# nordmtr/quantpy

Hardware: AMD Instinct MI355X
Metric: state reconstructions/sec (3-qubit MLE) (higher is better)
Workload: dtype f64

## Files before the change

quantpy_amd/csrc/qt_small.h:

```cpp
#pragma once
#include <hip/hip_runtime.h>
#include <stdint.h>

#include <type_traits>

#include "qt_linesearch.h"

namespace qt {

#ifdef QT_PHASE_TIMING
__device__ long long* g_qt_prof = nullptr;
#define QT_STAMP(slot)                                                                                   \
  do {                                                                                                   \
    if (g_qt_prof && (threadIdx.x & 63) == 0)                                                            \
      g_qt_prof[((size_t)blockIdx.x * (blockDim.x >> 6) + (threadIdx.x >> 6)) * 32 + (slot)] =           \
          (long long)__builtin_readcyclecounter();                                                       \
  } while (0)
#define QT_STAMP_VAL(slot, val)                                                                          \
  do {                                                                                                   \
    if (g_qt_prof && (threadIdx.x & 63) == 0)                                                            \
      g_qt_prof[((size_t)blockIdx.x * (blockDim.x >> 6) + (threadIdx.x >> 6)) * 32 + (slot)] = (val);    \
  } while (0)
#else
#define QT_STAMP(slot) do {} while (0)
#define QT_STAMP_VAL(slot, val) do {} while (0)
#endif

struct alignas(16) cd {
  double re, im;
};
__device__ __forceinline__ cd cmul(cd a, cd b) { return {a.re * b.re - a.im * b.im, a.re * b.im + a.im * b.re}; }
__device__ __forceinline__ cd cmulc(cd a, cd b) {
  return {a.re * b.re + a.im * b.im, a.im * b.re - a.re * b.im};
}
__device__ __forceinline__ cd cadd(cd a, cd b) { return {a.re + b.re, a.im + b.im}; }
__device__ __forceinline__ cd hs_term(cd a, cd b) {
  return {__builtin_fma(a.re, b.re, -(a.im * b.im)), __builtin_fma(a.re, b.im, a.im * b.re)};
}
__device__ __forceinline__ cd cscale(cd a, double s) { return {a.re * s, a.im * s}; }

__device__ __forceinline__ void wave_sync() {
  __builtin_amdgcn_wave_barrier();
  asm volatile("" ::: "memory");
}

template <int CTRL, int ROW_MASK = 0xf>
__device__ __forceinline__ double dpp_f64(double v) {
  const long long b = __builtin_bit_cast(long long, v);
  const int lo = __builtin_amdgcn_update_dpp(0, (int)(b & 0xffffffffLL), CTRL, ROW_MASK, 0xf, ROW_MASK == 0xf);
  const int hi = __builtin_amdgcn_update_dpp(0, (int)(b >> 32), CTRL, ROW_MASK, 0xf, ROW_MASK == 0xf);
  return __builtin_bit_cast(double, ((long long)hi << 32) | (unsigned int)lo);
}
__device__ __forceinline__ double readlane_f64(double v, int lane) {
  const long long b = __builtin_bit_cast(long long, v);
  const int lo = __builtin_amdgcn_readlane((int)(b & 0xffffffffLL), lane);
  const int hi = __builtin_amdgcn_readlane((int)(b >> 32), lane);
  return __builtin_bit_cast(double, ((long long)hi << 32) | (unsigned int)lo);
}
__device__ __forceinline__ double nanmax(double a, double b) { return (b > a || b != b) ? b : a; }

template <int G>
__device__ __forceinline__ double gsum(double v) {
  v += dpp_f64<0xB1>(v);
  v += dpp_f64<0x4E>(v);
  if (G >= 8) v += dpp_f64<0x141>(v);
  if (G >= 16) v += dpp_f64<0x140>(v);
  if (G == 64) {
    v += dpp_f64<0x142, 0xA>(v);
    v += dpp_f64<0x143, 0xC>(v);
    v = readlane_f64(v, 63);
  }
  return v;
}
template <int G>
__device__ __forceinline__ bool group_any(bool pred) {
  const unsigned long long votes = __builtin_amdgcn_ballot_w64(pred);
  if (G == 64) return votes != 0ull;
  const int lane = threadIdx.x & 63;
  return (votes & (((1ull << (G & 63)) - 1ull) << (lane / G * G))) != 0ull;
}
__device__ __forceinline__ double max_f64(double a, double b) {
  double r;
  asm("v_max_f64 %0, %1, %2" : "=v"(r) : "v"(a), "v"(b));
  return r;
}
template <int G>
__device__ __forceinline__ double gmax(double v) {
  const bool nan = group_any<G>(v != v);
  v = max_f64(v, dpp_f64<0xB1>(v));
  v = max_f64(v, dpp_f64<0x4E>(v));
  if (G >= 8) v = max_f64(v, dpp_f64<0x141>(v));
  if (G >= 16) v = max_f64(v, dpp_f64<0x140>(v));
  if (G == 64) {
    v = max_f64(v, dpp_f64<0x142, 0xA>(v));
    v = max_f64(v, dpp_f64<0x143, 0xC>(v));
    v = readlane_f64(v, 63);
  }
  return nan ? __builtin_nan("") : v;
}

__device__ __forceinline__ double recip_nr(double x) {
  double r = __builtin_amdgcn_rcp(x);
  r = fma(r, fma(-x, r, 1.0), r);
  return fma(r, fma(-x, r, 1.0), r);
}
__device__ __forceinline__ bool log_is_regular(double x) { return x > 0.0 && x < 1.7e308; }
__device__ __forceinline__ double fast_log(double x) {
  if (!(x > 0.0) || !(x < 1.7e308)) return x == 0.0 ? -__builtin_huge_val() : (x > 0.0 ? x : __builtin_nan(""));
  double m = __builtin_amdgcn_frexp_mant(x);
  int e = __builtin_amdgcn_frexp_exp(x);
  const bool low = m < 0.70710678118654752440;
  m = low ? m + m : m;
  e = low ? e - 1 : e;
  const double num = m - 1.0, den = m + 1.0;
  const double r = recip_nr(den);
  double sq = num * r;
  sq = fma(r, fma(-sq, den, num), sq);
  const double z = sq * sq;
  const double z2 = z * z, z4 = z2 * z2, z8 = z4 * z4;
  const double q0 = fma(z, 1.0 / 5.0, 1.0 / 3.0), q1 = fma(z, 1.0 / 9.0, 1.0 / 7.0);
  const double q2 = fma(z, 1.0 / 13.0, 1.0 / 11.0), q3 = fma(z, 1.0 / 17.0, 1.0 / 15.0);
  const double q4 = fma(z, 1.0 / 21.0, 1.0 / 19.0);
  const double r0 = fma(z2, q1, q0), r1 = fma(z2, q3, q2);
  const double pl = fma(z8, q4, fma(z4, r1, r0));
  const double lm = fma(sq + sq, pl * z, sq + sq);
  const double ed = (double)e;
  return fma(ed, 6.93147180369123816490e-01, fma(ed, 1.90821492927058770002e-10, lm));
}

constexpr bool kLiftSingleNegative = true;

__device__ __forceinline__ double fast_rsqrt(double x) {
  double y = __builtin_amdgcn_rsq(x);
  double e = fma(-x * y, y, 1.0);
  y = fma(y * e, fma(e, 0.375, 0.5), y);
  e = fma(-x * y, y, 1.0);
  return fma(y * e, 0.5, y);
}

template <int UNR>
__device__ __forceinline__ void dot_block(const double* __restrict__ base, size_t stride, unsigned lane_off,
                                          const double* lds_vec, int m, double (&acc)[4]) {
  double av[UNR];
#pragma unroll
  for (int u = 0; u < UNR; ++u) av[u] = base[(size_t)(m + u) * stride + lane_off];
#pragma unroll
  for (int u = 0; u < UNR; ++u) acc[u & 3] = fma(av[u], lds_vec[m + u], acc[u & 3]);
  __builtin_amdgcn_sched_group_barrier(0x020, UNR, 0);
#pragma unroll
  for (int u = 0; u < UNR; u += 4) {
    __builtin_amdgcn_sched_group_barrier(0x100, 2, 0);
    __builtin_amdgcn_sched_group_barrier(0x002, 4, 0);
  }
}
template <int UNR>
__device__ __forceinline__ double dot_global(const double* __restrict__ base, size_t stride, unsigned lane_off,
                                             const double* lds_vec, int n) {
  double acc[4] = {0.0, 0.0, 0.0, 0.0};
  int m = 0;
  for (; m + UNR <= n; m += UNR) dot_block<UNR>(base, stride, lane_off, lds_vec, m, acc);
  if (UNR > 8 && m + 8 <= n) {
    dot_block<8>(base, stride, lane_off, lds_vec, m, acc);
    m += 8;
  }
  if (UNR > 4 && m + 4 <= n) {
    dot_block<4>(base, stride, lane_off, lds_vec, m, acc);
    m += 4;
  }
  for (; m < n; ++m) acc[0] = fma(base[(size_t)m * stride + lane_off], lds_vec[m], acc[0]);
  return (acc[0] + acc[1]) + (acc[2] + acc[3]);
}

__device__ __forceinline__ void rotation(double app, double aqq, cd apq, double& cs, cd& w) {
  const double ab2 = apq.re * apq.re + apq.im * apq.im;
  cs = 1.0;
  w = cd{0.0, 0.0};
  if (ab2 > 1e-300) {
    const double dl = 0.5 * (aqq - app);
    const double x = fma(dl, dl, ab2);
    double y = __builtin_amdgcn_rsq(x);
    y = fma(y * fma(-x * y, y, 1.0), 0.5, y);
    const double den = fabs(dl) + x * y;
    double z = __builtin_amdgcn_rcp(den);
    z = fma(z, fma(-den, z, 1.0), z);
    const double u = copysign(z, dl);
    cs = fast_rsqrt(fma(u * u, ab2, 1.0));
    const double cu = cs * u;
    w = cd{cu * apq.re, cu * apq.im};
  }
}


struct ProductView {
  const double* T;
  const double* P1T;
  const double* wrowR;
  const int* rmap;
  const int* rinv;
  const int* fwd;
  const int* bwd;
  int R1;
  int uniform;
  double wuni;
  int enabled;
  int pairedT, pairedP;
  double cT[12], cP[12];
  const int* last;
};

struct PovmView {
  const double* Aw;
  const double* AwT;
  const double* PinvT;
  int M;
  ProductView pr;
  double jtol2 = 1e-28;
  const double* Ns = nullptr;
  int S = 0, K = 0;
  double ns_tot = 0.0;
  int extra = 0;
};

struct SpecArgs {
  const void* image;
  const double* Ns;
  double ns_tot, wuni, jtol2;
  int M, extra;
  double cT[12], cP[12];
};
template <bool GENERIC>
struct MleArgs {
  using type = PovmView;
};
template <>
struct MleArgs<false> {
  using type = SpecArgs;
};

__device__ __forceinline__ bool shots_match(double t_s, double total, double n_s, double ns_tot) {
  const double a = t_s * ns_tot, b = n_s * total;
  return fabs(a - b) <= 2e-15 * fabs(b);
}

struct EstOut {
  double* rho;
  const double* centre;
  double* dist;
};

template <int NQ>
struct Small {
  static constexpr int d = 1 << NQ;
  static constexpr int D = d * d;
  static constexpr int G = D;
  static constexpr int TPW = 64 / G;
  static constexpr int WPB = 4;
  static constexpr int NT = 64 * WPB;
  static constexpr int TPB = TPW * WPB;
  static constexpr int T = d * (d - 1) / 2;
  static constexpr int LD = d == 8 ? 9 : d;
  static constexpr int MAT = 2 * LD * d;
  static constexpr int oA = 0;
  static constexpr int oB = oA + MAT;
  static constexpr int oVec = oB + MAT;
  static constexpr int oLam = oVec + D + 2;
  static constexpr int oM = oLam + 2 * ((d + 1) / 2);
  __host__ __device__ static bool v_on_rbuf(int M) { return ((M + 1) & ~1) >= MAT; }
  __host__ __device__ static int v_offset(int M, int R1) {
    const int Mp = (M + 1) & ~1;
    return v_on_rbuf(M) ? oM : oM + (R1 > 0 ? 3 : 2) * Mp;
  }
  __host__ __device__ static int trial_doubles(int M, int R1 = 0) {
    const int Mp = (M + 1) & ~1;
    return oM + (R1 > 0 ? 3 : 2) * Mp + (v_on_rbuf(M) ? 0 : MAT);
  }
  __host__ __device__ static int ipow_h(int b, int e) {
    int r = 1;
    for (int t = 0; t < e; ++t) r *= b;
    return r;
  }
  __host__ __device__ static int fwd_ints(int R1) {
    int t = 0;
    for (int q = 1; q <= NQ; ++q) t += ipow_h(R1, q) << (2 * (NQ - q));
    return t;
  }
  __host__ __device__ static int bwd_ints(int R1) {
    int t = 0;
    for (int q = 1; q <= NQ; ++q) t += ipow_h(R1, q - 1) << (2 * (NQ - q + 1));
    return t;
  }
  __host__ __device__ static int table_ints(int M, int R1) { return (fwd_ints(R1) + bwd_ints(R1) + M + 1) & ~1; }
  __host__ __device__ static int table_doubles(int M, int R1) {
    return R1 > 0 ? (table_ints(M, R1) / 2 + ((M + 1) & ~1) + 8 * R1) : 0;
  }
  __host__ __device__ static size_t lds_bytes(int M, int R1 = 0, int extra = 0) {
    return ((size_t)table_doubles(M, R1) + (size_t)TPB * (trial_doubles(M, R1) + extra)) * sizeof(double);
  }

  struct Ctx {
    int l, i, j, e;
    double* sm;
    const int *tfwd, *tbwd, *trmap;
    const double* twrow;
    const double *ttab, *ptab;
    int M, Mp;
    PovmView pv;
    int xm, zm, ny;
    int pi, pj, pkind;
    int src_re, src_im;
    __device__ __forceinline__ cd* A() const { return reinterpret_cast<cd*>(sm + oA); }
    __device__ __forceinline__ cd* Bm() const { return reinterpret_cast<cd*>(sm + oB); }
    __device__ __forceinline__ cd* V() const { return reinterpret_cast<cd*>(sm + v_offset(M, pv.pr.enabled ? pv.pr.R1 : 0)); }
    __device__ __forceinline__ double* vec() const { return sm + oVec; }
    __device__ __forceinline__ double* lam() const { return sm + oLam; }
    __device__ __forceinline__ double* rbuf() const { return sm + oM; }
    __device__ __forceinline__ double* freq() const { return sm + oM + Mp; }
    __device__ __forceinline__ double* bufB() const { return sm + oM + 2 * Mp; }
    __device__ __forceinline__ const double* tabT() const { return ttab; }
    __device__ __forceinline__ const double* tabP() const { return ptab; }
    __device__ __forceinline__ bool prod() const { return pv.pr.enabled != 0; }
    __device__ __forceinline__ double* extra() const { return sm + trial_doubles(M, pv.pr.enabled ? pv.pr.R1 : 0); }
    static constexpr bool kGeneric = true;
    static constexpr bool kHelper = false;
    __device__ __forceinline__ int R1() const { return pv.pr.R1; }
    __device__ __forceinline__ bool uniform() const { return pv.pr.uniform != 0; }
    __device__ __forceinline__ bool pairedT() const { return pv.pr.pairedT != 0; }
    __device__ __forceinline__ bool pairedP() const { return pv.pr.pairedP != 0; }
    __device__ __forceinline__ double wuni() const { return pv.pr.wuni; }
    __device__ __forceinline__ double jtol2() const { return pv.jtol2; }
    __device__ __forceinline__ double cT(int k) const { return pv.pr.cT[k]; }
    __device__ __forceinline__ double cP(int k) const { return pv.pr.cP[k]; }
  };
  struct CtxS {
    int l, i, j, e;
    double* sm;
    const int* tfwd;
    const double *ttab, *ptab;
    int M, Mp;
    SpecArgs a;
    int xm, zm, ny;
    int pi, pj, pkind;
    int src_re, src_im;
    int bslot;
    double kT[12], kP[12];
    __device__ __forceinline__ cd* A() const { return reinterpret_cast<cd*>(sm + oA); }
    __device__ __forceinline__ cd* Bm() const { return reinterpret_cast<cd*>(sm + oB); }
    __device__ __forceinline__ cd* V() const { return reinterpret_cast<cd*>(sm + v_offset(M, 6)); }
    __device__ __forceinline__ double* vec() const { return sm + oVec; }
    __device__ __forceinline__ double* lam() const { return sm + oLam; }
    __device__ __forceinline__ double* rbuf() const { return sm + oM; }
    __device__ __forceinline__ double* freq() const { return sm + oM + Mp; }
    __device__ __forceinline__ double* bufB() const { return sm + oM + 2 * Mp; }
    __device__ __forceinline__ const double* tabT() const { return ttab; }
    __device__ __forceinline__ const double* tabP() const { return ptab; }
    __device__ __forceinline__ double* extra() const { return sm + trial_doubles(M, 6); }
    static constexpr bool kGeneric = false;
    static constexpr bool kHelper = false;
    __device__ __forceinline__ static constexpr bool prod() { return true; }
    __device__ __forceinline__ static constexpr int R1() { return 6; }
    __device__ __forceinline__ static constexpr bool uniform() { return true; }
    __device__ __forceinline__ static constexpr bool pairedT() { return true; }
    __device__ __forceinline__ static constexpr bool pairedP() { return true; }
    __device__ __forceinline__ double wuni() const { return a.wuni; }
    __device__ __forceinline__ double jtol2() const { return a.jtol2; }
    __device__ __forceinline__ double cT(int k) const { return kT[k]; }
    __device__ __forceinline__ double cP(int k) const { return kP[k]; }
  };
  __device__ __forceinline__ static double pin_vgpr(double x) {
    asm volatile("" : "+v"(x));
    return x;
  }
  template <bool GENERIC, class = void>
  struct CtxOf {
    using type = Ctx;
  };
  template <class X>
  struct CtxOf<false, X> {
    using type = CtxS;
  };
  __host__ __device__ static int image_last_ints(int M) { return (M + 3) & ~3; }
  __host__ __device__ static int image_chunks(int M) { return image_last_ints(M) / 4 + 2 * 24 / 2; }

  __device__ __forceinline__ static int trial_index(int B, bool* live) {
    const int wave = threadIdx.x >> 6, tib = (threadIdx.x & 63) / G;
    const int b = (blockIdx.x * WPB + wave) * TPW + tib;
    *live = b < B;
    return b;
  }

  __device__ static void make_ctx(Ctx& c, double* smem_block, const PovmView& pv) {
    const int lane = threadIdx.x & 63, wave = threadIdx.x >> 6;
    c.l = lane % G;
    const int slot = wave * TPW + lane / G;
    c.i = c.l / d;
    c.j = c.l % d;
    c.e = c.i * LD + c.j;
    c.M = pv.M;
    c.Mp = (pv.M + 1) & ~1;
    c.pv = pv;
    const int r1 = pv.pr.enabled ? pv.pr.R1 : 0;
    int* tabs = reinterpret_cast<int*>(smem_block);
    c.tfwd = tabs;
    c.tbwd = tabs + fwd_ints(r1);
    c.trmap = c.tbwd + bwd_ints(r1);
    double* wrow = smem_block + table_ints(pv.M, r1) / 2;
    double* t1 = wrow + ((pv.M + 1) & ~1);
    c.twrow = wrow;
    c.ttab = t1;
    c.ptab = t1 + 4 * r1;
    if (r1 > 0) {
      const int nf = fwd_ints(r1), nb = bwd_ints(r1);
      for (int e = threadIdx.x; e < 4 * r1; e += NT) {
        t1[e] = pv.pr.T[e];
        t1[4 * r1 + e] = pv.pr.P1T[e];
      }
      if (pv.pr.pairedT) {
        for (int e = threadIdx.x; e < pv.M; e += NT) tabs[e] = pv.pr.last[e];
      } else {
        for (int e = threadIdx.x; e < nf; e += NT) tabs[e] = pv.pr.fwd[e];
      }
      if (!(pv.pr.pairedT && pv.pr.pairedP))
        for (int e = threadIdx.x; e < nb; e += NT) tabs[nf + e] = pv.pr.bwd[e];
      for (int e = threadIdx.x; e < pv.M; e += NT) {
        tabs[nf + nb + e] = pv.pr.rmap[e];
        wrow[e] = pv.pr.wrowR[e];
      }
      __syncthreads();
    }
    c.sm = smem_block + table_doubles(pv.M, r1) + slot * (trial_doubles(pv.M, r1) + pv.extra);
    int xm = 0, zm = 0, ny = 0;
#pragma unroll
    for (int b = 0; b < NQ; ++b) {
      const int dig = (c.l >> (2 * b)) & 3;
      if (dig == 1 || dig == 2) xm |= 1 << b;
      if (dig == 2 || dig == 3) zm |= 1 << b;
      if (dig == 2) ++ny;
    }
    c.xm = xm;
    c.zm = zm;
    c.ny = ny & 3;
    if (c.l < d) {
      c.pi = c.pj = c.l;
      c.pkind = 0;
    } else {
      int t = c.l - d;
      c.pkind = 1;
      if (t >= T) {
        t -= T;
        c.pkind = 2;
      }
      int ii = 1;
      while ((ii * (ii + 1)) / 2 <= t) ++ii;
      c.pi = ii;
      c.pj = t - (ii * (ii - 1)) / 2;
    }
    c.src_re = c.src_im = D;
    if (c.i == c.j) c.src_re = c.i;
    else if (c.i > c.j) {
      const int tt = (c.i * (c.i - 1)) / 2 + c.j;
      c.src_re = d + tt;
      c.src_im = d + T + tt;
    }
    if (c.l == 0) c.sm[oVec + D] = 0.0;
  }

  __device__ __forceinline__ static int pauli_index(int x, int z) {
    int k = 0;
#pragma unroll
    for (int b = 0; b < NQ; ++b) {
      const int xb = (x >> b) & 1, zb = (z >> b) & 1;
      const int dig = xb ? (zb ? 2 : 1) : (zb ? 3 : 0);
      k |= dig << (2 * b);
    }
    return k;
  }
  __device__ __forceinline__ static double re_phase(int ny, cd s) {
    return ny == 0 ? s.re : ny == 1 ? s.im : ny == 2 ? -s.re : -s.im;
  }
  __device__ __forceinline__ static cd phase_times(int ny, double v) {
    return ny == 0 ? cd{v, 0.0} : ny == 1 ? cd{0.0, -v} : ny == 2 ? cd{-v, 0.0} : cd{0.0, v};
  }

  __device__ __forceinline__ static cd wht_step(cd s, cd p, bool upper) {
    return upper ? cd{p.re - s.re, p.im - s.im} : cd{s.re + p.re, s.im + p.im};
  }
  template <class C>
  __device__ static double bloch_of(const C& c, const cd* m) {
    if constexpr (NQ == 3) {
      const int x = c.i, r = c.j, lane = threadIdx.x & 63;
      const cd e = m[r * LD + (r ^ x)];
      cd s{e.re, -e.im};
      s = wht_step(s, cd{dpp_f64<0xB1>(s.re), dpp_f64<0xB1>(s.im)}, lane & 1);
      s = wht_step(s, cd{dpp_f64<0x4E>(s.re), dpp_f64<0x4E>(s.im)}, lane & 2);
      s = wht_step(s, cd{__shfl_xor(s.re, 4), __shfl_xor(s.im, 4)}, lane & 4);
      const int z = r;
      const double v = re_phase(__popc(x & z) & 3, s) / d;
      const int sx = (x & 1) | ((x & 2) << 1) | ((x & 4) << 2), sz = (z & 1) | ((z & 2) << 1) | ((z & 4) << 2);
      double* vec = c.vec();
      if constexpr (C::kGeneric) vec[sx ^ (3 * sz)] = v;
      else vec[c.bslot] = v;
      wave_sync();
      const double mine = vec[c.l];
      wave_sync();
      return mine;
    }
    cd s{0.0, 0.0};
#pragma unroll
    for (int r = 0; r < d; ++r) {
      const cd e = m[r * LD + (r ^ c.xm)];
      const double sg = (__popc(r & c.zm) & 1) ? -1.0 : 1.0;
// ... 464 lines not shown
    return dot_global<(D < 16 ? D : 16)>(g_transposed, (size_t)c.M, (unsigned)row, vec, D);
  }

  template <class C>
  __device__ static cd lin_invert(const C& c, double& bloch_l) {
    if constexpr (!C::kGeneric) {
      bloch_l = prod_backward<true>(c, c.freq()) / (c.wuni() * d);
    } else if (c.prod()) {
      if (c.uniform()) {
        bloch_l = prod_backward<true>(c, c.freq()) / (c.wuni() * d);
      } else {
        double acc = 0.0;
        for (int m = 0; m < c.M; ++m) acc = fma(c.pv.PinvT[(size_t)c.trmap[m] * D + c.l], c.freq()[m], acc);
        bloch_l = acc / d;
      }
    } else {
      bloch_l = col_dot(c, c.pv.PinvT, c.freq()) / d;
    }
    c.vec()[c.l] = bloch_l;
    wave_sync();
    cd r = matrix_of(c, c.vec());
    wave_sync();
    return r;
  }

  template <class C>
  __device__ static cd psd_project(const C& c, cd a, double eps) {
    const int i = c.i, j = c.j;
    cd* Ai = c.A();
    cd* Vi = c.V();
    cd v{i == j ? 1.0 : 0.0, 0.0};
    if (i == j) a.im = 0.0;
    const double nrm = gsum<G>(a.re * a.re + a.im * a.im);
    for (int sweep = 0; sweep < 20; ++sweep) {
      const double off = gsum<G>(i != j ? a.re * a.re + a.im * a.im : 0.0);
      if (__all(!(off > c.jtol2() * nrm))) break;
#pragma unroll 1
      for (int r = 1; r < d; ++r) {
        Ai[c.e] = a;
        Vi[c.e] = v;
        wave_sync();
        const int pj = j ^ r, pi = i ^ r;
        const int cp = j < pj ? j : pj, cq = j < pj ? pj : j;
        const int rp = i < pi ? i : pi, rq = i < pi ? pi : i;
        const double c_pp = Ai[cp * LD + cp].re, c_qq = Ai[cq * LD + cq].re;
        const cd c_pq = Ai[cp * LD + cq];
        const double r_pp = Ai[rp * LD + rp].re, r_qq = Ai[rq * LD + rq].re;
        const cd r_pq = Ai[rp * LD + rq];
        const cd a_c = Ai[i * LD + pj], a_r = Ai[pi * LD + j], a_x = Ai[pi * LD + pj];
        const cd v_c = Vi[i * LD + pj];
        wave_sync();
        double cj, ci;
        cd wj, wi;
        rotation(c_pp, c_qq, c_pq, cj, wj);
        rotation(r_pp, r_qq, r_pq, ci, wi);
        if (j < pj) wj = cd{-wj.re, wj.im};
        if (i < pi) wi = cd{-wi.re, wi.im};
        const cd t0 = cadd(cscale(a, cj), cmul(a_c, wj));
        const cd t1 = cadd(cscale(a_r, cj), cmul(a_x, wj));
        a = cadd(cscale(t0, ci), cmulc(t1, wi));
        v = cadd(cscale(v, cj), cmul(v_c, wj));
        if (i == j) a.im = 0.0;
      }
    }
    double* lam = c.lam();
    Vi[c.e] = v;
    if (i == j) lam[i] = a.re;
    wave_sync();
    cd rr{0.0, 0.0};
#pragma unroll
    for (int k = 0; k < d; ++k) {
      const double lc = lam[k] > eps ? lam[k] : eps;
      const cd p = cmulc(Vi[i * LD + k], Vi[j * LD + k]);
      rr.re += lc * p.re;
      rr.im += lc * p.im;
    }
    const double tr = gsum<G>(i == j ? rr.re : 0.0);
    wave_sync();
    return cd{rr.re / tr, rr.im / tr};
  }

  template <bool SPEC = false, class C>
  __device__ static double cholesky_param(const C& c, cd a, int& ok, int* neg_out = nullptr, int* kneg_out = nullptr,
                                          cd* spec_inv = nullptr) {
    cd* A = c.A();
    cd* L = c.Bm();
    cd* Vs = c.V();
    const int i = c.i, j = c.j;
    A[c.e] = a;
    int neg = 0, kneg = d - 1;
    cd lmine{0.0, 0.0};
    cd b = a;
    if (SPEC && i == j) b.im = 0.0;
    if (SPEC) Vs[c.e] = b;
    wave_sync();
#pragma unroll
    for (int k = 0; k < d; ++k) {
      const double akk = (G == 64) ? readlane_f64(a.re, k * d + k) : A[k * LD + k].re;
      const cd aik = A[i * LD + k], ajk = A[j * LD + k];
      if constexpr (SPEC) {
        const double piv = readlane_f64(b.re, k * d + k);
        const cd bip = Vs[i * LD + k], bpj = Vs[k * LD + j];
        double inv = __builtin_amdgcn_rcp(piv);
        inv = fma(inv, fma(-piv, inv, 1.0), inv);
        inv = fma(inv, fma(-piv, inv, 1.0), inv);
        const cd t{bpj.re * inv, bpj.im * inv};
        const cd e = cmul(bip, t);
        cd nb{b.re - e.re, b.im - e.im};
        if (j == k) nb = cd{-bip.re * inv, -bip.im * inv};
        if (i == k) nb = (j == k) ? cd{inv, 0.0} : t;
        b = nb;
        if (k + 1 < d) Vs[c.e] = b;
      }
      const double mag = fabs(akk);
      const bool pos = akk > 0.0;
      if (!pos) {
        if (neg == 0) kneg = k;
        ++neg;
      }
      if (!(mag > 1e-13)) neg = neg > 0 ? 99 : neg;
      const double safe = mag > 1e-300 ? mag : 1e-300;
      if (k + 1 < d) {
        const double inv = recip_nr(safe);
        const double sinv = pos ? -inv : inv;
        const cd ajs{ajk.re * sinv, ajk.im * sinv};
        const bool upd = i > k && j > k;
        const double nre = fma(aik.re, ajs.re, fma(aik.im, ajs.im, a.re));
        const double nim = fma(aik.im, ajs.re, fma(-aik.re, ajs.im, a.im));
        a.re = upd ? nre : a.re;
        a.im = upd ? nim : a.im;
        A[c.e] = a;
        wave_sync();
      }
    }
    {
      const double dj = A[j * LD + j].re;
      const double mj = fabs(dj);
      const double rs = fast_rsqrt(mj > 1e-300 ? mj : 1e-300);
      if (i >= j) lmine = (i == j) ? cd{dj * rs, 0.0} : cd{a.re * rs, a.im * rs};
    }
    ok = neg == 0;
    if (neg_out) *neg_out = neg;
    if (kneg_out) *kneg_out = kneg;
    if (SPEC && spec_inv) *spec_inv = b;
    L[c.e] = lmine;
    wave_sync();
    const cd e = L[c.pi * LD + c.pj];
    const double x = c.pkind == 2 ? e.im : e.re;
    wave_sync();
    return x;
  }

  struct HelperLink {
    enum : int { kNone = 0, kSweep = 1, kUnset = 2, kClaimed = 3, kRevoked = 4 };
    static constexpr int kHelperPolls = 1 << 15, kWaitPolls = 1 << 12, kClaimedPolls = 1 << 16;
    double* base;
    int pending;
    __device__ __forceinline__ static constexpr int doubles() { return MAT + D + 2; }
    __device__ __forceinline__ cd* image() const { return reinterpret_cast<cd*>(base); }
    __device__ __forceinline__ double* x() const { return base + MAT; }
    __device__ __forceinline__ int* task() const { return reinterpret_cast<int*>(base + MAT + D); }
    __device__ __forceinline__ int* done() const { return task() + 1; }
    __device__ __forceinline__ int* ok() const { return task() + 2; }
    __device__ __forceinline__ static void publish(int* w, int v) {
      wave_sync();
      if ((threadIdx.x & 63) == 0) __hip_atomic_store(w, v, __ATOMIC_RELEASE, __HIP_MEMORY_SCOPE_WORKGROUP);
    }
    __device__ __forceinline__ static int peek(const int* w) {
      return __builtin_amdgcn_readfirstlane(__hip_atomic_load(w, __ATOMIC_RELAXED, __HIP_MEMORY_SCOPE_WORKGROUP));
    }
    __device__ __forceinline__ static bool claim(int* w, int to) {
      int won = 0;
      if ((threadIdx.x & 63) == 0) {
        int expect = kSweep;
        won = __hip_atomic_compare_exchange_strong(w, &expect, to, __ATOMIC_ACQ_REL, __ATOMIC_RELAXED,
                                                   __HIP_MEMORY_SCOPE_WORKGROUP);
      }
      return __builtin_amdgcn_readfirstlane(won) != 0;
    }
    template <int SLEEP>
    __device__ __forceinline__ static int poll(const int* w, int idle, int polls) {
      int v = idle;
#pragma unroll 1
      for (int n = 0; n < polls; ++n) {
        v = peek(w);
        if (v != idle) break;
        __builtin_amdgcn_s_sleep(SLEEP);
      }
      return v;
    }
    __device__ __forceinline__ void reset() {
      pending = 0;
      if ((threadIdx.x & 63) == 0) {
        *task() = kUnset;
        *done() = 0;
      }
    }
    __device__ __forceinline__ void none() const { publish(task(), kNone); }
    __device__ __forceinline__ void give(int e, cd proj) {
      image()[e] = proj;
      publish(task(), kSweep);
      pending = 1;
    }
    __device__ __forceinline__ bool collect(int l, double& xl, int& okl) const {
      if (poll<1>(done(), 0, kWaitPolls) == 0) {
        if (claim(task(), kRevoked)) return false;
        if (poll<1>(done(), 0, kClaimedPolls) == 0) return false;
      }
      __builtin_amdgcn_fence(__ATOMIC_ACQUIRE, "workgroup");
      xl = x()[l];
      okl = *ok();
      return true;
    }
  };
  struct CtxH {
    int l, i, j, e, pi, pj, pkind;
    cd *image, *factor;
    __device__ __forceinline__ cd* A() const { return image; }
    __device__ __forceinline__ cd* Bm() const { return factor; }
    __device__ __forceinline__ cd* V() const { return nullptr; }
  };
  struct LateX {
    bool got;
    double x;
    int ok;
  };
  template <class Base>
  struct WithHelper : Base {
    HelperLink* link;
    LateX* late;
    static constexpr bool kHelper = true;
  };
  __device__ __forceinline__ static void param_owner(int l, int& pi, int& pj, int& pkind) {
    const bool diag = l < d, imag = l >= d + T;
    const int t = l - d - (imag ? T : 0);
    int ii = 1;
#pragma unroll
    for (int k = 2; k < d; ++k) ii += t >= (k * (k - 1)) / 2;
    pkind = diag ? 0 : imag ? 2 : 1;
    pi = diag ? l : ii;
    pj = diag ? l : t - (ii * (ii - 1)) / 2;
  }
  __device__ static void helper_wave(const HelperLink& k, cd* L) {
    static_assert(G == 64, "one trial per wavefront");
    if (HelperLink::template poll<2>(k.task(), HelperLink::kUnset, HelperLink::kHelperPolls) != HelperLink::kSweep) return;
    if (!HelperLink::claim(k.task(), HelperLink::kClaimed)) return;
    __builtin_amdgcn_fence(__ATOMIC_ACQUIRE, "workgroup");
    CtxH c;
    c.l = threadIdx.x & 63;
    c.i = c.l / d;
    c.j = c.l % d;
    c.e = c.i * LD + c.j;
    param_owner(c.l, c.pi, c.pj, c.pkind);
    c.image = k.image();
    c.factor = L;
    int ok2;
    const double x2 = cholesky_param(c, c.image[c.e], ok2);
    k.x()[c.l] = x2;
    if (c.l == 0) *k.ok() = ok2;
    HelperLink::publish(k.done(), 1);
  }

  template <class C>
  __device__ static bool lift_single_negative(const C& c, cd r, int kneg, double eps, cd& out,
                                              const cd* inverse = nullptr) {
    static_assert(G == 64, "one trial per wavefront: the flags below are wave-uniform");
    cd* Ai = c.A();
    cd* Vi = c.V();
    const int i = c.i, j = c.j;
    if (i == j) r.im = 0.0;
    cd b = r;
    if (inverse) b = *inverse;
#pragma unroll 1
    for (int s = inverse ? d : 0; s < d; ++s) {
      const int p = s < kneg ? s : (s < d - 1 ? s + 1 : kneg);
      Ai[c.e] = b;
      const double piv = readlane_f64(b.re, p * d + p);
      wave_sync();
      const cd bip = Ai[i * LD + p], bpj = Ai[p * LD + j];
      wave_sync();
      double inv = __builtin_amdgcn_rcp(piv);
      inv = fma(inv, fma(-piv, inv, 1.0), inv);
      inv = fma(inv, fma(-piv, inv, 1.0), inv);
      const cd t{bpj.re * inv, bpj.im * inv};
      const cd e = cmul(bip, t);
      cd nb{b.re - e.re, b.im - e.im};
      if (j == p) nb = cd{-bip.re * inv, -bip.im * inv};
      if (i == p) nb = (j == p) ? cd{inv, 0.0} : t;
      b = nb;
    }
    QT_STAMP(4);
    b = cscale(b, fast_rsqrt(gsum<G>(b.re * b.re + b.im * b.im)));
    bool certified = false, done = false;
#pragma unroll 1
    for (int k = 1; k <= 7 && !done; ++k) {
      Ai[c.e] = b;
      wave_sync();
      cd n{0.0, 0.0}, n2{0.0, 0.0};
#pragma unroll
      for (int q = 0; q < d; q += 2) {
        const cd u = Ai[i * LD + q], v = Ai[j * LD + q];
        n.re = fma(u.re, v.re, fma(u.im, v.im, n.re));
        n.im = fma(u.im, v.re, fma(-u.re, v.im, n.im));
        if (q + 1 < d) {
          const cd u2 = Ai[i * LD + q + 1], v2 = Ai[j * LD + q + 1];
          n2.re = fma(u2.re, v2.re, fma(u2.im, v2.im, n2.re));
          n2.im = fma(u2.im, v2.re, fma(-u2.re, v2.im, n2.im));
        }
      }
      n = cadd(n, n2);
      wave_sync();
      const double pur = gsum<G>(n.re * n.re + n.im * n.im);
      b = cscale(n, fast_rsqrt(pur));
      const double defect = 1.0 - pur;
      QT_STAMP_VAL(20, k);
      if (certified) done = true;
      else if (defect < 1e-7) certified = true;
      else if (k == 3 && !(defect < 0.05)) return false;
    }
    QT_STAMP(5);
    if (!done) return false;
    if (i == j) b.im = 0.0;
    b = cscale(b, 1.0 / gsum<G>(i == j ? b.re : 0.0));
    const double lam = gsum<G>(r.re * b.re + r.im * b.im);
    if (!(lam < eps)) return false;
    Ai[c.e] = r;
    Vi[c.e] = b;
    wave_sync();
    cd q{-lam * b.re, -lam * b.im};
#pragma unroll
    for (int k = 0; k < d; ++k) {
      const cd u = Ai[i * LD + k], v = Vi[j * LD + k];
      q.re = fma(u.re, v.re, fma(u.im, v.im, q.re));
      q.im = fma(u.im, v.re, fma(-u.re, v.im, q.im));
    }
    wave_sync();
    const double res2 = gsum<G>(q.re * q.re + q.im * q.im);
    const double nrm2 = gsum<G>(r.re * r.re + r.im * r.im);
    if (!(res2 <= 1e-26 * nrm2)) return false;
    const double w = eps - lam;
    cd o{fma(w, b.re, r.re), fma(w, b.im, r.im)};
    const double tr = gsum<G>(i == j ? o.re : 0.0);
    out = cd{o.re / tr, o.im / tr};
    return true;
  }

  template <bool SPEC = false, class C>
  __device__ static cd make_feasible(const C& c, cd r, double* xl, int* ok_out, double* lscale_out = nullptr) {
    int ok, neg, kneg;
    cd spec_inv{0.0, 0.0};
    double x = cholesky_param<SPEC && G == 64>(c, r, ok, &neg, &kneg, &spec_inv);
    QT_STAMP(3);
    cd out{0.0, 0.0};
    double lscale = 1.0;
    auto pd_epilogue = [&]() {
      const double tr = gsum<G>(c.i == c.j ? r.re : 0.0);
      out = cd{r.re / tr, r.im / tr};
      const double rst = tr > 0.0 ? fast_rsqrt(tr) : 1.0 / sqrt(tr);
      x = x * rst;
      lscale = rst;
    };
    const bool all_pd = __all(ok);
    if constexpr (C::kHelper) {
      if (all_pd) c.link->none();
    }
    if (G < 64 || all_pd || (!xl && lscale_out)) pd_epilogue();
    if (!all_pd) {
      cd proj;
      bool lifted = false;
      if constexpr (G == 64) {
        if (kLiftSingleNegative && __builtin_amdgcn_readfirstlane(neg) == 1) {
          const int kn = __builtin_amdgcn_readfirstlane(kneg);
          lifted = __builtin_amdgcn_readfirstlane(
                       (int)lift_single_negative(c, r, kn, 1e-15, proj, SPEC && kn == d - 1 ? &spec_inv : nullptr)) != 0;
        }
      }
      if constexpr (C::kHelper) {
        if (!lifted) c.link->none();
      }
      if (!lifted) proj = psd_project(c, r, 1e-15);
      QT_STAMP(6);
      if constexpr (C::kHelper) {
        if (lifted) {
          c.link->give(c.e, proj);
          if (lscale_out) *lscale_out = 1.0;
          return proj;
        }
      }
      int ok2 = 1;
      double x2 = xl ? cholesky_param(c, proj, ok2) : 0.0;
      if (lifted && xl && !__all(ok2 || ok)) {
        proj = psd_project(c, r, 1e-15);
        x2 = cholesky_param(c, proj, ok2);
      }
      QT_STAMP(7);
      if (xl) lscale = 1.0;
      if (!ok) {
        out = proj;
        x = x2;
        ok = ok2;
      }
    }
    if (xl) *xl = x;
    if (ok_out) *ok_out = ok;
    if (lscale_out) *lscale_out = lscale;
    return out;
  }

  template <class C>
  __device__ static cd build_llh(const C& c, double xl, double& tr) {
    double* vx = c.vec();
    cd* L = c.Bm();
    vx[c.l] = xl;
    tr = gsum<G>(xl * xl);
    wave_sync();
    const int i = c.i, j = c.j;
    L[c.e] = cd{vx[c.src_re], vx[c.src_im]};
    wave_sync();
    cd m{0.0, 0.0};
#pragma unroll
    for (int k = 0; k < d; ++k) {
      const cd u = L[i * LD + k], v = L[j * LD + k];
      m.re = fma(u.re, v.re, fma(u.im, v.im, m.re));
      m.im = fma(u.im, v.re, fma(-u.re, v.im, m.im));
    }
    return m;
  }

  struct StartPoint {
    cd rho;
    double lscale;
  };
  template <bool DEFER = false, class C, bool LATE = false>
  __device__ static void nll_grad(const C& c, double xl, double& f, double& gl, cd* rho_l = nullptr,
                                  bool want_grad = true, const StartPoint* start = nullptr, DeferredValue* dv = nullptr) {
    static_assert(!DEFER || !C::kGeneric, "the deferred value needs the compile-time row count of the specialised shape");
    double tr;
    QT_STAMP(11);
    cd m;
    if constexpr (LATE) {
      m = start->rho;
    } else if (start) {
      tr = gsum<G>(xl * xl);
      m = cd{start->rho.re * tr, start->rho.im * tr};
    } else {
      m = build_llh(c, xl, tr);
    }
    QT_STAMP(12);
    cd* A = c.A();
    const cd rho_e = start ? start->rho : cd{m.re / tr, m.im / tr};
    if (rho_l) *rho_l = rho_e;
    A[c.e] = rho_e;
    wave_sync();
    const double bl = bloch_of(c, A);
    QT_STAMP(13);
    double* vec = c.vec();
    vec[c.l] = bl;
    wave_sync();
    double fpart = 0.0;
    const double* fr = c.freq();
    double* rb = c.rbuf();
    double wl;
    if (c.prod()) {
      const int R1 = c.R1();
      const bool paired = c.pairedT() != 0;
      const int* tab = c.tfwd;
      const double* in = vec;
#pragma unroll
      for (int q = 1; q < NQ; ++q) {
        const int stride = 1 << (2 * (NQ - q));
        const int n_out = ipow(R1, q) * stride;
        double* out = ((NQ - 1 - q) & 1) ? rb : c.bufB();
        if (paired) {
          paired_forward(c, q, in, out);
        } else if constexpr (C::kGeneric) {
          stage<true>(c, c.tabT(), tab, n_out, stride, in, out);
          tab += n_out;
        }
        in = out;
      }
      QT_STAMP(14);
      if constexpr (DEFER) {
        stage_n_log<true, true, true>(c, tab, in, fr, rb, dv);
      } else if constexpr (!C::kGeneric) {
        fpart = stage_n_log<true, true>(c, tab, in, fr, rb);
      } else {
        if (!paired) fpart = stage_n_log<false, false>(c, tab, in, fr, rb);
        else if (c.uniform()) fpart = stage_n_log<true, true>(c, tab, in, fr, rb);
        else fpart = stage_n_log<true, false>(c, tab, in, fr, rb);
      }
      if constexpr (!DEFER) f = -gsum<G>(fpart);
      wave_sync();
      QT_STAMP(15);
      if (!want_grad) return;
      wl = prod_backward<false>(c, rb);
      QT_STAMP(16);
    } else if constexpr (C::kGeneric) {
      for (int m0 = 0; m0 < c.M; m0 += G) {
        const int mm = m0 + c.l;
        if (mm < c.M) {
          const double pe = row_dot(c, c.pv.AwT, mm, vec) * d + 1e-10;
          fpart += fr[mm] * fast_log(pe);
          rb[mm] = fr[mm] * recip_nr(pe);
        }
      }
      f = -gsum<G>(fpart);
      wave_sync();
      if (!want_grad) return;
      wl = col_dot(c, c.pv.Aw, rb);
    }
    const double tr_g_rho = -(double)d * gsum<G>(wl * bl);
    vec[c.l] = wl;
    wave_sync();
    cd g = matrix_of(c, vec);
    QT_STAMP(17);
    if constexpr (LATE) {
      LateX& lx = *c.late;
      lx.x = 1.0;
      lx.ok = 0;
      lx.got = c.link->collect(c.l, lx.x, lx.ok);
      xl = lx.x;
      tr = gsum<G>(xl * xl);
      QT_STAMP(25);
    }
    g.re = -g.re;
    g.im = -g.im;
    if (c.i == c.j) g.re -= tr_g_rho;
    g.re /= tr;
    g.im /= tr;
    A[c.e] = g;
    wave_sync();
    const cd* L = c.Bm();
    cd q{0.0, 0.0};
#pragma unroll
    for (int k = 0; k < d; ++k) {
      const cd u = A[c.pi * LD + k], v = L[k * LD + c.pj];
      q.re = fma(u.re, v.re, fma(-u.im, v.im, q.re));
      q.im = fma(u.re, v.im, fma(u.im, v.re, q.im));
    }
    gl = 2.0 * (c.pkind == 2 ? q.im : q.re);
    if (start) gl *= start->lscale;
// ... 377 lines not shown
          }
          if (c.l == 0) prho[np] = rhok;
          wave_sync();
          double q = gk;
          for (int i = np; i >= 0; --i) {
            double si = sk, yi = yk;
            if (i != np) {
              if (i < LP) {
                si = lp[(2 * i) * D];
                yi = lp[(2 * i + 1) * D];
              } else {
                si = my[(size_t)(2 * i) * D];
                yi = my[(size_t)(2 * i + 1) * D];
              }
            }
            const double a = prho[i] * gsum<G>(si * q);
            if (c.l == 0) palpha[i] = a;
            q = fma(-a, yi, q);
          }
          wave_sync();
          for (int i = 0; i <= np; ++i) {
            double si = sk, yi = yk;
            if (i != np) {
              if (i < LP) {
                si = lp[(2 * i) * D];
                yi = lp[(2 * i + 1) * D];
              } else {
                si = my[(size_t)(2 * i) * D];
                yi = my[(size_t)(2 * i + 1) * D];
              }
            }
            const double bb = prho[i] * gsum<G>(yi * q);
            q = fma(si, palpha[i] - bb, q);
          }
          pk = -q;
          ls.start(fk, old_old, gsum<G>(gk * pk), &stp);
        }
      }
    }
    wave_sync();
  }
  if (status == 0) {
    const double gn = gmax<G>(fabs(gk));
    const double xn = gmax<G>(fabs(xk));
    if (kiter >= max_iter) status = 3;
    else if (gn != gn || fk != fk || xn != xn) status = 4;
  }
  double tr;
  const cd m = S::build_llh(c, xk, tr);
  S::emit(c, rho, b, mine, cd{m.re / tr, m.im / tr});
  if (mine) {
    if (c.l == 0) {
      if (nit_out) nit_out[b] = kiter;
      if (nfev_out) nfev_out[b] = nfev;
      if (fun_out) fun_out[b] = fk;
      if (status_out) status_out[b] = status;
    }
  }
}

#ifndef QT_BFGS_WAVES
#define QT_BFGS_WAVES 2
#endif
template <int NQ, bool GENERIC>
__global__ void __launch_bounds__(256) __attribute__((amdgpu_waves_per_eu(QT_BFGS_WAVES))) k_mle_bfgs(typename MleArgs<GENERIC>::type pv, const int64_t* __restrict__ counts, int B, int max_iter,
                                                  double gtol, EstOut rho, int32_t* __restrict__ nit_out,
                                                  int32_t* __restrict__ nfev_out, double* __restrict__ fun_out,
                                                  int32_t* __restrict__ status_out, const double* __restrict__ ws_x,
                                                  const double* __restrict__ ws_g, const double* __restrict__ ws_f,
                                                  const int32_t* __restrict__ ws_active, double* __restrict__ pairs) {
  using S = Small<NQ>;
  constexpr int D = S::D;
  bool live;
  const int b = S::trial_index(B, &live);
  const bool mine = live && ws_active[b] != 0;
  if (!__syncthreads_or(mine)) return;
  extern __shared__ __attribute__((aligned(16))) double smem[];
  typename S::template CtxOf<GENERIC>::type c;
  const int bb = live ? b : B - 1;
  if constexpr (GENERIC) {
    S::make_ctx(c, smem, pv);
    S::load_freq(c, counts + (size_t)bb * pv.M);
  } else {
    typename S::Prefetch pf;
    S::prefetch_counts(pf, counts + (size_t)bb * pv.M, pv);
    S::make_ctx(c, smem, pv, pf);
    S::load_freq(c, pf);
  }
  const double xk = mine ? ws_x[(size_t)b * D + c.l] : (c.l < S::d ? 1.0 : 0.0);
  const double gk = mine ? ws_g[(size_t)b * D + c.l] : 0.0;
  const double fk = mine ? ws_f[b] : 0.0;
  if constexpr (NQ == 3)
    bfgs_iterate_2l<NQ>(c, mine, xk, gk, fk, b, max_iter, gtol, rho, nit_out, nfev_out, fun_out, status_out, pairs);
  else
    bfgs_iterate<NQ>(c, mine, xk, gk, fk, b, max_iter, gtol, rho, nit_out, nfev_out, fun_out, status_out);
}

constexpr int kFusedLdsPairs = 24;

template <int NQ, bool GENERIC, bool HW = false>
__device__ __forceinline__ void mle_fused_body(const typename MleArgs<GENERIC>::type& pv, const int64_t* __restrict__ counts, int B, int init,
                                               int max_iter, double gtol, EstOut rho,
                                               int32_t* __restrict__ nit_out, int32_t* __restrict__ nfev_out,
                                               double* __restrict__ fun_out, int32_t* __restrict__ status_out,
                                               double* __restrict__ pairs) {
  using S = Small<NQ>;
  constexpr int D = S::D, G = S::G, d = S::d;
  extern __shared__ __attribute__((aligned(16))) double smem[];
  using Ctx = typename S::template CtxOf<GENERIC>::type;
  std::conditional_t<HW, typename S::template WithHelper<Ctx>, Ctx> c;
  [[maybe_unused]] typename S::HelperLink link;
  [[maybe_unused]] typename S::LateX late{false, 0.0, 0};
  if constexpr (HW) {
    static_assert(NQ == 3, "one trial per wavefront");
    static_assert(S::HelperLink::doubles() <= kFusedLdsPairs * 2 * D, "the hand-off lives in the LDS pair store");
    int r1 = 6;
    if constexpr (GENERIC) r1 = pv.pr.R1;
    const int per_trial = S::trial_doubles(pv.M, r1);
    double* sm = smem + S::table_doubles(pv.M, r1) + (threadIdx.x >> 6) * (per_trial + pv.extra);
    link.base = sm + per_trial + LineSearch::SLOTS + 2 * max_iter;
    if (__builtin_amdgcn_readfirstlane((int)threadIdx.y) != 0) {
      __syncthreads();
      S::helper_wave(link, reinterpret_cast<cd*>(sm + S::oB));
      return;
    }
    link.reset();
    c.link = &link;
    c.late = &late;
  }
  bool live;
  const int b = S::trial_index(B, &live);
  const int bb = live ? b : B - 1;
  typename S::Prefetch pf;
  S::prefetch_counts(pf, counts + (size_t)bb * pv.M, pv);
  bool shots_ok;
  if constexpr (GENERIC) {
    S::make_ctx(c, smem, pv);
    QT_STAMP(0);
    shots_ok = S::load_freq(c, counts + (size_t)bb * pv.M, &pf);
  } else {
    S::template make_ctx<true>(c, smem, pv, pf);
    QT_STAMP(0);
    shots_ok = S::load_freq(c, pf);
  }
  QT_STAMP(1);
  int ok;
  double xk;
  typename S::StartPoint sp;
  [[maybe_unused]] cd lin;
  if (init == 0) {
    double bl;
    lin = S::lin_invert(c, bl);
    QT_STAMP(2);
    sp.rho = S::template make_feasible<true>(c, lin, &xk, &ok, &sp.lscale);
  } else {
    sp.rho = cd{c.i == c.j ? 1.0 / d : 0.0, 0.0};
    sp.lscale = 1.0;
    xk = S::cholesky_param(c, sp.rho, ok);
  }
  QT_STAMP(8);
  double fk, gk;
  cd rho_l;
  [[maybe_unused]] typename S::DeferredValue dv;
  bool evaluate = true;
  if constexpr (HW) {
    if (__builtin_amdgcn_readfirstlane(link.pending)) {
      if constexpr (GENERIC) S::template nll_grad<false, decltype(c), true>(c, 0.0, fk, gk, &rho_l, true, &sp);
      else S::template nll_grad<true, decltype(c), true>(c, 0.0, fk, gk, &rho_l, true, &sp, &dv);
      xk = late.x;
      ok = late.ok;
      const bool got = __builtin_amdgcn_readfirstlane((int)late.got) != 0;
      if (!got) xk = S::cholesky_param(c, sp.rho, ok);
      ok = __builtin_amdgcn_readfirstlane(ok);
      evaluate = !got || !ok;
      if (!ok) {
        sp.rho = S::psd_project(c, lin, 1e-15);
        xk = S::cholesky_param(c, sp.rho, ok);
      }
    }
  }
  if (evaluate) {
    if constexpr (GENERIC) S::nll_grad(c, xk, fk, gk, &rho_l, true, &sp);
    else S::template nll_grad<true>(c, xk, fk, gk, &rho_l, true, &sp, &dv);
  }
  const double gnorm = gmax<G>(fabs(gk));
  QT_STAMP(9);
  const bool iterate = live && shots_ok && ok && (gnorm > gtol) && (0 < max_iter);
  if constexpr (!GENERIC) fk = S::value_if_needed(c, dv, iterate || fun_out != nullptr);
  S::emit(c, rho, b, live && !iterate, rho_l);
  if (!iterate) {
    int status = 0;
    if (!shots_ok) status = 5;
    else if (!ok) status = 1;
    else {
      const bool xnan = group_any<G>(xk != xk);
      if (0 >= max_iter) status = 3;
      else if (gnorm != gnorm || fk != fk || xnan) status = 4;
    }
    if (live) {
      if (c.l == 0) {
        if (nit_out) nit_out[b] = 0;
        if (nfev_out) nfev_out[b] = ok ? 1 : 0;
        if (fun_out) fun_out[b] = fk;
        if (status_out) status_out[b] = status;
      }
    }
  }
  QT_STAMP(10);
  if (!__any(iterate)) return;
  if (!iterate) {
    xk = (c.l < d) ? 1.0 : 0.0;
    gk = 0.0;
    fk = 0.0;
  }
  if constexpr (NQ == 3)
    bfgs_iterate_2l<NQ, kFusedLdsPairs>(c, iterate, xk, gk, fk, b, max_iter, gtol, rho, nit_out, nfev_out, fun_out,
                                              status_out, pairs);
  else
    bfgs_iterate<NQ>(c, iterate, xk, gk, fk, b, max_iter, gtol, rho, nit_out, nfev_out, fun_out, status_out);
}

template <int NQ, bool GENERIC>
__global__ void __launch_bounds__(256) k_mle_fused(typename MleArgs<GENERIC>::type pv, const int64_t* __restrict__ counts, int B, int max_iter,
                                                   double gtol, EstOut rho, int32_t* __restrict__ nit_out,
                                                   int32_t* __restrict__ nfev_out, double* __restrict__ fun_out,
                                                   int32_t* __restrict__ status_out, double* __restrict__ pairs) {
  mle_fused_body<NQ, GENERIC>(pv, counts, B, 0, max_iter, gtol, rho, nit_out, nfev_out, fun_out, status_out, pairs);
}
template <int NQ, bool GENERIC>
__global__ void __launch_bounds__(256) k_mle_fused_mixed(typename MleArgs<GENERIC>::type pv, const int64_t* __restrict__ counts, int B,
                                                         int max_iter, double gtol, EstOut rho,
                                                         int32_t* __restrict__ nit_out, int32_t* __restrict__ nfev_out,
                                                         double* __restrict__ fun_out, int32_t* __restrict__ status_out,
                                                         double* __restrict__ pairs) {
  mle_fused_body<NQ, GENERIC>(pv, counts, B, 1, max_iter, gtol, rho, nit_out, nfev_out, fun_out, status_out, pairs);
}

template <int NQ, bool GENERIC>
__global__ void __launch_bounds__(512) k_mle_fused_hw(typename MleArgs<GENERIC>::type pv, const int64_t* __restrict__ counts, int B, int max_iter,
                                                      double gtol, EstOut rho, int32_t* __restrict__ nit_out,
                                                      int32_t* __restrict__ nfev_out, double* __restrict__ fun_out,
                                                      int32_t* __restrict__ status_out, double* __restrict__ pairs) {
  mle_fused_body<NQ, GENERIC, true>(pv, counts, B, 0, max_iter, gtol, rho, nit_out, nfev_out, fun_out, status_out, pairs);
}

template <int NQ>
__global__ void __launch_bounds__(256) k_mhmc_state(PovmView pv, const int64_t* __restrict__ counts, int C,
                                                    const double* __restrict__ x_init, const double* __restrict__ deltas,
                                                    const double* __restrict__ uniforms, int T_steps, double step,
                                                    double* __restrict__ chain, int32_t* __restrict__ accepted) {
  using S = Small<NQ>;
  constexpr int D = S::D, G = S::G;
  extern __shared__ __attribute__((aligned(16))) double smem[];
  typename S::Ctx c;
  S::make_ctx(c, smem, pv);
  bool live;
  const int b = S::trial_index(C, &live);
  const int bb = live ? b : C - 1;
  S::load_freq(c, counts + (size_t)bb * pv.M);
  double x = x_init[(size_t)bb * D + c.l];
  double f, unused;
  S::nll_grad(c, x, f, unused, nullptr, false);
  const double* dl = deltas + (size_t)bb * T_steps * D + c.l;
  const double* un = uniforms + (size_t)bb * T_steps;
  for (int t = 0; t < T_steps; ++t) {
    const double xp = fma(step, dl[(size_t)t * D], x);
    const double nrm = sqrt(gsum<G>(xp * xp));
    const double xn = xp / nrm;
    double fn;
    S::nll_grad(c, xn, fn, unused, nullptr, false);
    const double alpha = exp(f - fn);
    const bool acc = un[t] <= alpha;
    if (acc) {
      x = xn;
      f = fn;
    }
    if (live) {
      chain[((size_t)b * T_steps + t) * D + c.l] = x;
      if (c.l == 0) accepted[(size_t)b * T_steps + t] = acc ? 1 : 0;
    }
  }
}

}
```

Measured before the change: 96.72 million.

## Speculatively start helper-wave negative-eigenvalue lift before main wave decides

The helper wavefront now receives the linear-inversion estimate right after lin_invert and computes the single-negative-eigenvalue lift speculatively, while the main wave runs its own Cholesky/PSD check. The main wave then publishes a go/abort verdict and, on go, waits for the helper's lifted projection instead of computing it itself. An abandonment check inside the lift iteration lets the helper stop early when aborted, and the main wave waits for the helper to finish before BFGS. This moves the lift off the critical path, at the cost of more LDS for a second image, extra polling and handshake state, and wasted helper work when the speculation is not needed.

```diff
diff --git a/quantpy_amd/csrc/qt_small.h b/quantpy_amd/csrc/qt_small.h
--- a/quantpy_amd/csrc/qt_small.h
+++ b/quantpy_amd/csrc/qt_small.h
@@ -10,16 +10,17 @@
 
 #ifdef QT_PHASE_TIMING
 __device__ long long* g_qt_prof = nullptr;
+#define QT_PROF_ROW \
+  ((size_t)(blockIdx.x + threadIdx.y * gridDim.x) * (blockDim.x >> 6) + (threadIdx.x >> 6))
 #define QT_STAMP(slot)                                                                                   \
   do {                                                                                                   \
     if (g_qt_prof && (threadIdx.x & 63) == 0)                                                            \
-      g_qt_prof[((size_t)blockIdx.x * (blockDim.x >> 6) + (threadIdx.x >> 6)) * 32 + (slot)] =           \
-          (long long)__builtin_readcyclecounter();                                                       \
+      g_qt_prof[QT_PROF_ROW * 32 + (slot)] = (long long)__builtin_readcyclecounter();                    \
   } while (0)
 #define QT_STAMP_VAL(slot, val)                                                                          \
   do {                                                                                                   \
     if (g_qt_prof && (threadIdx.x & 63) == 0)                                                            \
-      g_qt_prof[((size_t)blockIdx.x * (blockDim.x >> 6) + (threadIdx.x >> 6)) * 32 + (slot)] = (val);    \
+      g_qt_prof[QT_PROF_ROW * 32 + (slot)] = (val);                                                      \
   } while (0)
 #else
 #define QT_STAMP(slot) do {} while (0)
@@ -322,6 +323,8 @@
     __device__ __forceinline__ double* extra() const { return sm + trial_doubles(M, pv.pr.enabled ? pv.pr.R1 : 0); }
     static constexpr bool kGeneric = true;
     static constexpr bool kHelper = false;
+    __device__ __forceinline__ static constexpr int verdict_load() { return 0; }
+    __device__ __forceinline__ static constexpr bool abandoned(int) { return false; }
     __device__ __forceinline__ int R1() const { return pv.pr.R1; }
     __device__ __forceinline__ bool uniform() const { return pv.pr.uniform != 0; }
     __device__ __forceinline__ bool pairedT() const { return pv.pr.pairedT != 0; }
@@ -356,6 +359,8 @@
     __device__ __forceinline__ double* extra() const { return sm + trial_doubles(M, 6); }
     static constexpr bool kGeneric = false;
     static constexpr bool kHelper = false;
+    __device__ __forceinline__ static constexpr int verdict_load() { return 0; }
+    __device__ __forceinline__ static constexpr bool abandoned(int) { return false; }
     __device__ __forceinline__ static constexpr bool prod() { return true; }
     __device__ __forceinline__ static constexpr int R1() { return 6; }
     __device__ __forceinline__ static constexpr bool uniform() { return true; }
@@ -1126,16 +1131,22 @@
   }
 
   struct HelperLink {
-    enum : int { kNone = 0, kSweep = 1, kUnset = 2, kClaimed = 3, kRevoked = 4 };
-    static constexpr int kHelperPolls = 1 << 15, kWaitPolls = 1 << 12, kClaimedPolls = 1 << 16;
+    enum : int { kUnset = 0, kSpec = 1 };
+    enum : int { kPending = 0, kGo = 1, kAbort = 2, kClaimed = 3, kRevoked = 4 };
+    enum : int { kNothing = 0, kLifted = 1, kRefused = 2 };
+    static constexpr int kHelperPolls = 1 << 15, kWaitPolls = 1 << 14, kClaimedPolls = 1 << 16;
     double* base;
     int pending;
-    __device__ __forceinline__ static constexpr int doubles() { return MAT + D + 2; }
-    __device__ __forceinline__ cd* image() const { return reinterpret_cast<cd*>(base); }
-    __device__ __forceinline__ double* x() const { return base + MAT; }
-    __device__ __forceinline__ int* task() const { return reinterpret_cast<int*>(base + MAT + D); }
-    __device__ __forceinline__ int* done() const { return task() + 1; }
-    __device__ __forceinline__ int* ok() const { return task() + 2; }
+    __device__ __forceinline__ static constexpr int doubles() { return 2 * MAT + D + 3; }
+    __device__ __forceinline__ cd* image(int k) const { return reinterpret_cast<cd*>(base + k * MAT); }
+    __device__ __forceinline__ cd* result() const { return image(1); }
+    __device__ __forceinline__ double* x() const { return base + 2 * MAT; }
+    __device__ __forceinline__ int* task() const { return reinterpret_cast<int*>(base + 2 * MAT + D); }
+    __device__ __forceinline__ int* verdict() const { return task() + 1; }
+    __device__ __forceinline__ int* lifted() const { return task() + 2; }
+    __device__ __forceinline__ int* done() const { return task() + 3; }
+    __device__ __forceinline__ int* gone() const { return task() + 4; }
+    __device__ __forceinline__ int* ok() const { return task() + 5; }
     __device__ __forceinline__ static void publish(int* w, int v) {
       wave_sync();
       if ((threadIdx.x & 63) == 0) __hip_atomic_store(w, v, __ATOMIC_RELEASE, __HIP_MEMORY_SCOPE_WORKGROUP);
@@ -1143,10 +1154,10 @@
     __device__ __forceinline__ static int peek(const int* w) {
       return __builtin_amdgcn_readfirstlane(__hip_atomic_load(w, __ATOMIC_RELAXED, __HIP_MEMORY_SCOPE_WORKGROUP));
     }
-    __device__ __forceinline__ static bool claim(int* w, int to) {
+    __device__ __forceinline__ static bool claim(int* w, int from, int to) {
       int won = 0;
       if ((threadIdx.x & 63) == 0) {
-        int expect = kSweep;
+        int expect = from;
         won = __hip_atomic_compare_exchange_strong(w, &expect, to, __ATOMIC_ACQ_REL, __ATOMIC_RELAXED,
                                                    __HIP_MEMORY_SCOPE_WORKGROUP);
       }
@@ -1167,32 +1178,57 @@
       pending = 0;
       if ((threadIdx.x & 63) == 0) {
         *task() = kUnset;
+        *verdict() = kPending;
+        *lifted() = kNothing;
         *done() = 0;
-      }
-    }
-    __device__ __forceinline__ void none() const { publish(task(), kNone); }
-    __device__ __forceinline__ void give(int e, cd proj) {
-      image()[e] = proj;
-      publish(task(), kSweep);
-      pending = 1;
+        *gone() = 0;
+      }
+    }
+    __device__ __forceinline__ void speculate(int e, cd lin) const {
+      image(0)[e] = lin;
+      publish(task(), kSpec);
+    }
+    __device__ __forceinline__ void decide(bool go) const { publish(verdict(), go ? kGo : kAbort); }
+    __device__ __forceinline__ int await_lift(int e, cd& proj) {
+      int v = poll<1>(lifted(), kNothing, kWaitPolls);
+      if (v == kNothing) {
+        if (claim(verdict(), kGo, kRevoked)) return kNothing;
+        v = poll<1>(lifted(), kNothing, kClaimedPolls);
+        if (v == kNothing) return kNothing;
+      }
+      __builtin_amdgcn_fence(__ATOMIC_ACQUIRE, "workgroup");
+      if (v == kLifted) {
+        proj = result()[e];
+        pending = 1;
+      }
+      return v;
     }
     __device__ __forceinline__ bool collect(int l, double& xl, int& okl) const {
-      if (poll<1>(done(), 0, kWaitPolls) == 0) {
-        if (claim(task(), kRevoked)) return false;
-        if (poll<1>(done(), 0, kClaimedPolls) == 0) return false;
-      }
+      if (poll<1>(done(), 0, kClaimedPolls) == 0) return false;
       __builtin_amdgcn_fence(__ATOMIC_ACQUIRE, "workgroup");
       xl = x()[l];
       okl = *ok();
       return true;
     }
+    __device__ __forceinline__ void await_gone() const {
+      poll<1>(gone(), 0, kClaimedPolls);
+      __builtin_amdgcn_fence(__ATOMIC_ACQUIRE, "workgroup");
+    }
   };
   struct CtxH {
     int l, i, j, e, pi, pj, pkind;
-    cd *image, *factor;
+    cd *image, *second, *factor;
+    const int* verdict;
     __device__ __forceinline__ cd* A() const { return image; }
     __device__ __forceinline__ cd* Bm() const { return factor; }
-    __device__ __forceinline__ cd* V() const { return nullptr; }
+    __device__ __forceinline__ cd* V() const { return second; }
+    __device__ __forceinline__ int verdict_load() const {
+      return __hip_atomic_load(verdict, __ATOMIC_RELAXED, __HIP_MEMORY_SCOPE_WORKGROUP);
+    }
+    __device__ __forceinline__ static bool abandoned(int v) {
+      v = __builtin_amdgcn_readfirstlane(v);
+      return v != HelperLink::kPending && v != HelperLink::kGo;
+    }
   };
   struct LateX {
     bool got;
@@ -1216,23 +1252,43 @@
     pj = diag ? l : t - (ii * (ii - 1)) / 2;
   }
   __device__ static void helper_wave(const HelperLink& k, cd* L) {
+    helper_work(k, L);
+    HelperLink::publish(k.gone(), 1);
+  }
+  __device__ static void helper_work(const HelperLink& k, cd* L) {
     static_assert(G == 64, "one trial per wavefront");
-    if (HelperLink::template poll<2>(k.task(), HelperLink::kUnset, HelperLink::kHelperPolls) != HelperLink::kSweep) return;
-    if (!HelperLink::claim(k.task(), HelperLink::kClaimed)) return;
+    if (HelperLink::template poll<2>(k.task(), HelperLink::kUnset, HelperLink::kHelperPolls) != HelperLink::kSpec) return;
     __builtin_amdgcn_fence(__ATOMIC_ACQUIRE, "workgroup");
+    QT_STAMP(0);
     CtxH c;
     c.l = threadIdx.x & 63;
     c.i = c.l / d;
     c.j = c.l % d;
     c.e = c.i * LD + c.j;
     param_owner(c.l, c.pi, c.pj, c.pkind);
-    c.image = k.image();
+    c.image = k.image(0);
+    c.second = k.image(1);
     c.factor = L;
+    c.verdict = k.verdict();
+    cd proj{0.0, 0.0};
+    const bool lifted =
+        __builtin_amdgcn_readfirstlane((int)lift_single_negative(c, c.image[c.e], d - 1, 1e-15, proj, nullptr)) != 0;
+    QT_STAMP(6);
+    if (HelperLink::template poll<1>(k.verdict(), HelperLink::kPending, HelperLink::kHelperPolls) != HelperLink::kGo) return;
+    QT_STAMP(7);
+    if (!HelperLink::claim(k.verdict(), HelperLink::kGo, HelperLink::kClaimed)) return;
+    if (!lifted) {
+      HelperLink::publish(k.lifted(), HelperLink::kRefused);
+      return;
+    }
+    k.result()[c.e] = proj;
+    HelperLink::publish(k.lifted(), HelperLink::kLifted);
     int ok2;
-    const double x2 = cholesky_param(c, c.image[c.e], ok2);
+    const double x2 = cholesky_param(c, proj, ok2);
     k.x()[c.l] = x2;
     if (c.l == 0) *k.ok() = ok2;
     HelperLink::publish(k.done(), 1);
+    QT_STAMP(8);
   }
 
   template <class C>
@@ -1270,6 +1326,7 @@
     for (int k = 1; k <= 7 && !done; ++k) {
       Ai[c.e] = b;
       wave_sync();
+      [[maybe_unused]] const int verdict = c.verdict_load();
       cd n{0.0, 0.0}, n2{0.0, 0.0};
 #pragma unroll
       for (int q = 0; q < d; q += 2) {
@@ -1284,10 +1341,14 @@
       }
       n = cadd(n, n2);
       wave_sync();
+      if (c.abandoned(verdict)) return false;
       const double pur = gsum<G>(n.re * n.re + n.im * n.im);
       b = cscale(n, fast_rsqrt(pur));
       const double defect = 1.0 - pur;
       QT_STAMP_VAL(20, k);
+#ifdef QT_PHASE_TIMING
+      if (k <= 5) QT_STAMP(25 + k);
+#endif
       if (certified) done = true;
       else if (defect < 1e-7) certified = true;
       else if (k == 3 && !(defect < 0.05)) return false;
@@ -1335,32 +1396,38 @@
       lscale = rst;
     };
     const bool all_pd = __all(ok);
+    [[maybe_unused]] bool go = false;
     if constexpr (C::kHelper) {
-      if (all_pd) c.link->none();
+      go = kLiftSingleNegative && !all_pd && __builtin_amdgcn_readfirstlane(neg) == 1 &&
+           __builtin_amdgcn_readfirstlane(kneg) == d - 1;
+      c.link->decide(go);
     }
     if (G < 64 || all_pd || (!xl && lscale_out)) pd_epilogue();
     if (!all_pd) {
       cd proj;
       bool lifted = false;
+      [[maybe_unused]] bool refused = false;
+      if constexpr (C::kHelper) {
+        if (go) {
+          const int came = c.link->await_lift(c.e, proj);
+          QT_STAMP(31);
+          if (came == HelperLink::kLifted) {
+            QT_STAMP(6);
+            if (lscale_out) *lscale_out = 1.0;
+            return proj;
+          }
+          refused = came == HelperLink::kRefused;
+        }
+      }
       if constexpr (G == 64) {
-        if (kLiftSingleNegative && __builtin_amdgcn_readfirstlane(neg) == 1) {
+        if (kLiftSingleNegative && !refused && __builtin_amdgcn_readfirstlane(neg) == 1) {
           const int kn = __builtin_amdgcn_readfirstlane(kneg);
           lifted = __builtin_amdgcn_readfirstlane(
                        (int)lift_single_negative(c, r, kn, 1e-15, proj, SPEC && kn == d - 1 ? &spec_inv : nullptr)) != 0;
         }
       }
-      if constexpr (C::kHelper) {
-        if (!lifted) c.link->none();
-      }
       if (!lifted) proj = psd_project(c, r, 1e-15);
       QT_STAMP(6);
-      if constexpr (C::kHelper) {
-        if (lifted) {
-          c.link->give(c.e, proj);
-          if (lscale_out) *lscale_out = 1.0;
-          return proj;
-        }
-      }
       int ok2 = 1;
       double x2 = xl ? cholesky_param(c, proj, ok2) : 0.0;
       if (lifted && xl && !__all(ok2 || ok)) {
@@ -2044,7 +2111,8 @@
     double bl;
     lin = S::lin_invert(c, bl);
     QT_STAMP(2);
-    sp.rho = S::template make_feasible<true>(c, lin, &xk, &ok, &sp.lscale);
+    if constexpr (HW) link.speculate(c.e, lin);
+    sp.rho = S::template make_feasible<!HW>(c, lin, &xk, &ok, &sp.lscale);
   } else {
     sp.rho = cd{c.i == c.j ? 1.0 / d : 0.0, 0.0};
     sp.lscale = 1.0;
@@ -2105,6 +2173,7 @@
     gk = 0.0;
     fk = 0.0;
   }
+  if constexpr (HW) link.await_gone();
   if constexpr (NQ == 3)
     bfgs_iterate_2l<NQ, kFusedLdsPairs>(c, iterate, xk, gk, fk, b, max_iter, gtol, rho, nit_out, nfev_out, fun_out,
                                               status_out, pairs);
```

Measured after the change: 98.56 million, median of 6. +1.9%, better.
